# zfountas/deep-active-inference-mc

Hardware: AMD Instinct MI355X
Metric: EFE rollouts/sec (64x64 dSprites, 10 MC-samples, depth 5) (higher is better)
Workload: dtype f32; 1 GPU; calculate_G_repeated: 128 rows (32 roots x 4 actions) x depth 5 x 10 MC samples per GPU (BASELINE configs[1]) + action posterior; rows_per_gpu=128, samples=10, depth=5, parallelism=episodes sharded x1, weights replicated

## Files before the change

deep-active-inference-mc_amd/csrc/decoder.hip:

```cpp
#include <utility>
#include "mfma_pipe.h"

namespace efe {

template <class F, int... I> __device__ __forceinline__ void static_for_(F&& f, std::integer_sequence<int, I...>) { (f(std::integral_constant<int, I>{}), ...); }
template <int N, class F> __device__ __forceinline__ void static_for(F&& f) { static_for_(f, std::make_integer_sequence<int, N>{}); }

__host__ __device__ constexpr int w3_nch(int G) { return G == 4 ? 5 : 4; }
__host__ __device__ constexpr int w3_prod(int G, int c) {
    return G < 4 ? 5 * ((G >> 1) + 2 * (c >> 1)) + (G & 1) + 2 * (c & 1)
         : G == 4 ? (c < 2 ? 5 * (1 + 2 * c) + 4 : c < 4 ? 20 + 1 + 2 * (c - 2) : 24)
                  : (c < 2 ? 5 * (2 * c) + 4 : 20 + 2 * (c - 2));
}
__host__ __device__ constexpr bool w3_direct(int pp) { return f22_o1(pp / 5) < 0 && f22_o1(pp % 5) < 0; }
__host__ __device__ constexpr int w3_view(int pp) { return 3 * f22_view(pp / 5) + f22_view(pp % 5); }
__host__ __device__ constexpr int w3_mat(int pp) { return 4 * f22_wt(pp / 5) + f22_wt(pp % 5); }
__host__ __device__ constexpr bool w3_hits(int pp, int o) {
    const int r = o >> 2, c = o & 3, pr = pp / 5, pc = pp % 5;
    return (r == f22_o0(pr) || r == f22_o1(pr)) && (c == f22_o0(pc) || c == f22_o1(pc));
}
__host__ __device__ constexpr bool w3_seen(int G, int c, int o) {
    for (int g = 0; g < G; ++g)
        for (int k = 0; k < w3_nch(g); ++k) if (w3_hits(w3_prod(g, k), o)) return true;
    if (!w3_direct(w3_prod(G, c)))
        for (int k = 0; k < w3_nch(G); ++k)
            if ((w3_direct(w3_prod(G, k)) || k < c) && w3_hits(w3_prod(G, k), o)) return true;
    return false;
}
__host__ __device__ constexpr bool w3_uses_view(int G, int vi) {
    for (int k = 0; k < w3_nch(G); ++k) if (w3_view(w3_prod(G, k)) == vi) return true;
    return false;
}
__host__ __device__ constexpr bool f22_in(int a, int r) { return a == 0 ? r <= 1 : (a == 1 ? r == 1 : r >= 1); }
__host__ __device__ constexpr bool w3_reads(int G, int r, int c) {
    for (int vi = 0; vi < 9; ++vi) if (w3_uses_view(G, vi) && f22_in(vi / 3, r) && f22_in(vi % 3, c)) return true;
    return false;
}

template <int PD, bool LATE, bool OPAQUE, bool WRAP, class WF, class PX, class Piece>
__device__ __forceinline__ void f22_contract(f32x4 (&acc)[16], f32x4 (&aq)[PD][5], const f32x4 bias4, WF wf, PX px, Piece piece) {
    constexpr int NST = 24;
    auto sub = [](const f32x4 a, const f32x4 b) -> f32x4 { if constexpr (OPAQUE) return sub4(a, b); else return a - b; };
    auto add = [](const f32x4 a, const f32x4 b) -> f32x4 { if constexpr (OPAQUE) return add4(a, b); else return a + b; };
    auto view = [&](const f32x4 (&x)[9], int vi) -> f32x4 {
        const int va = vi / 3, vb = vi % 3;
        auto cv = [&](int i) -> f32x4 { return vb == 0 ? sub(x[3 * i], x[3 * i + 1]) : (vb == 1 ? x[3 * i + 1] : sub(x[3 * i + 2], x[3 * i + 1])); };
        return va == 0 ? sub(cv(0), cv(1)) : (va == 1 ? cv(1) : sub(cv(2), cv(1)));
    };
    const f32x4 zero4 = {};
    f32x4 tq[5], xr[9];
    static_for<9>([&](auto i) { if constexpr (w3_reads(0, i / 3, i % 3)) xr[i] = px(i / 3, i % 3, 0); });
    auto add_tmp = [&](auto gg) {
        constexpr int GG = decltype(gg)::value;
        static_for<w3_nch(GG)>([&](auto c) {
            constexpr int PP = w3_prod(GG, c);
            if constexpr (!w3_direct(PP))
                static_for<16>([&](auto o) {
                    if constexpr (w3_hits(PP, o)) {
                        if constexpr (w3_seen(GG, c, o)) acc[o] = add(acc[o], tq[c]);
                        else acc[o] = add(bias4, tq[c]);
                    }
                });
        });
    };
    static_for<NST>([&](auto stc) {
        constexpr int ST = decltype(stc)::value, G = ST >> 2, KC = ST & 3, GN = (ST + 1) >> 2, KN = (ST + 1) & 3;
        constexpr int SP = (ST + PD) % NST, GP = SP >> 2, KP = SP & 3;
        f32x4 vw[9], ac[5];
        static_for<9>([&](auto vi) { if constexpr (w3_uses_view(G, vi)) vw[vi] = view(xr, vi); });
#pragma unroll
        for (int c = 0; c < 5; ++c) ac[c] = aq[ST % PD][c];
        if constexpr (WRAP || ST + PD < NST)
            static_for<w3_nch(GP)>([&](auto c) { aq[ST % PD][c] = wf(w3_mat(w3_prod(GP, c)), KP, ST + PD >= NST); });
        if constexpr (ST + 1 < NST)
            static_for<9>([&](auto i) { if constexpr (w3_reads(GN, i / 3, i % 3)) xr[i] = px(i / 3, i % 3, KN); });
        if constexpr (LATE && KC == 0 && ST > 0) {
            __builtin_amdgcn_sched_barrier(0);
            add_tmp(std::integral_constant<int, (ST > 0 ? G - 1 : 0)>{});
        }
        prio_matrix();
        __builtin_amdgcn_sched_barrier(0);
#pragma unroll
        for (int e = 0; e < 4; ++e)
            static_for<w3_nch(G)>([&](auto c) {
                constexpr int PP = w3_prod(G, c);
                const float b = vw[w3_view(PP)][e], av = ac[c][e];
                if constexpr (w3_direct(PP)) {
                    constexpr int O = 4 * f22_o0(PP / 5) + f22_o0(PP % 5);
                    constexpr bool FIRST = KC == 0 && !w3_seen(G, c, O);
                    acc[O] = __builtin_amdgcn_mfma_f32_16x16x4f32(av, b, (FIRST && e == 0) ? bias4 : acc[O], 0, 0, 0);
                } else {
                    tq[c] = __builtin_amdgcn_mfma_f32_16x16x4f32(av, b, (KC == 0 && e == 0) ? zero4 : tq[c], 0, 0, 0);
                }
            });
        prio_nonmatrix();
        if constexpr (!LATE && KC == 3) add_tmp(std::integral_constant<int, G>{});
        piece(stc);
    });
    if constexpr (LATE) add_tmp(std::integral_constant<int, 5>{});
}

constexpr int DA_PS = 17;
constexpr int DA_BIAS = 273 * DA_PS;

__host__ __device__ constexpr int wino_i0(int a) { return a == 0 ? 0 : (a == 2 ? 2 : 1); }
__host__ __device__ constexpr int wino_i1(int a) { return a == 0 ? 2 : (a == 1 ? 2 : (a == 2 ? 1 : 3)); }
__host__ __device__ constexpr float wino_s1(int a) { return a == 1 ? 1.0f : -1.0f; }
__host__ __device__ constexpr float wino_at(int r, int a) { return r == 0 ? (a < 3 ? 1.0f : 0.0f) : (a == 0 ? 0.0f : (a == 1 ? 1.0f : -1.0f)); }

__device__ __forceinline__ float4 fma4(float s, const float4& x, const float4& y) {
    return make_float4(__builtin_fmaf(s, x.x, y.x), __builtin_fmaf(s, x.y, y.y), __builtin_fmaf(s, x.z, y.z), __builtin_fmaf(s, x.w, y.w));
}
template <int NR, int R0, int MASK>
__device__ __forceinline__ void wino_otrans(f32x16 (&out)[NR][2], const int a, const int b, const f32x16& m) {
#pragma unroll
    for (int r = 0; r < NR; ++r) {
        if (!((MASK >> r) & 1)) continue;
        const float car = wino_at(R0 + r, a);
#pragma unroll
        for (int c = 0; c < 2; ++c) {
            const float cbc = wino_at(c, b);
            if (cbc == 0.0f) continue;
            const float cf = car * cbc;
#pragma unroll
            for (int e = 0; e < 16; ++e) out[r][c][e] = __builtin_fmaf(cf, m[e], out[r][c][e]);
        }
    }
}
template <int NR, int R0, class Pix>
__device__ __forceinline__ void wino_l1(f32x16 (&out)[NR][2], const float4* __restrict__ U, const float4* sm, const int h,
                                        const int mt_, Pix pix) {
    constexpr int PD = 4;
    const unsigned ln = (threadIdx.x & 63u) * 16u;
    const __amdgpu_buffer_rsrc_t ur = wrsrc(U);
    int mt = mt_; asm volatile("" : "+s"(mt));
    constexpr int a_lo = NR == 2 ? 0 : R0, a_hi = NR == 2 ? 4 : R0 + 3;
    auto ufrag = [&](int a, int b, int kc) { return wfrag(ur, ln, (size_t)(((4 * a + b) * 2 + mt) * 8 + kc) * 64); };
    auto bases = [&](int a, int b, int (&pb)[4]) {
        const int i0 = wino_i0(a), i1 = wino_i1(a), j0 = wino_i0(b), j1 = wino_i1(b);
        pb[0] = pix(i0, j0); pb[1] = pix(i0, j1); pb[2] = pix(i1, j0); pb[3] = pix(i1, j1);
    };
    float4 aq[PD], raw[4];
    int pb[4];
#pragma unroll
    for (int p = 0; p < PD; ++p) aq[p] = ufrag(a_lo, 0, p);
    bases(a_lo, 0, pb);
#pragma unroll
    for (int q = 0; q < 4; ++q) raw[q] = sm[pb[q] + h];
    f32x16 xacc;
    const f32x16 zero = {};
    auto xi_row = [&](int a, auto mask) {
        const float s1 = wino_s1(a);
        const int an = a + 1 < a_hi ? a + 1 : a;
#pragma unroll
        for (int b = 0; b < 4; ++b) {
            const float t1 = wino_s1(b);
#pragma unroll
            for (int kc = 0; kc < 8; ++kc) {
                const float4 av = aq[kc % PD];
                aq[kc % PD] = (b * 8 + kc + PD < 32) ? ufrag(a, (b * 8 + kc + PD) >> 3, (kc + PD) & 7) : ufrag(an, 0, (kc + PD) & 7);
                const float4 c0 = fma4(s1, raw[2], raw[0]), c1 = fma4(s1, raw[3], raw[1]);
                const float4 v = fma4(t1, c1, c0);
                if (kc < 7) {
#pragma unroll
                    for (int q = 0; q < 4; ++q) raw[q] = sm[pb[q] + 2 * (kc + 1) + h];
                } else {
                    if (b < 3) bases(a, b + 1, pb);
                    else bases(an, 0, pb);
#pragma unroll
                    for (int q = 0; q < 4; ++q) raw[q] = sm[pb[q] + h];
                }
                prio_matrix();
                __builtin_amdgcn_sched_barrier(0);
                f32x16& x = xacc;
                x = __builtin_amdgcn_mfma_f32_32x32x2f32(av.x, v.x, kc == 0 ? zero : x, 0, 0, 0);
                x = __builtin_amdgcn_mfma_f32_32x32x2f32(av.y, v.y, x, 0, 0, 0);
                x = __builtin_amdgcn_mfma_f32_32x32x2f32(av.z, v.z, x, 0, 0, 0);
                x = __builtin_amdgcn_mfma_f32_32x32x2f32(av.w, v.w, x, 0, 0, 0);
                prio_nonmatrix();
            }
            wino_otrans<NR, R0, decltype(mask)::value>(out, a, b, xacc);
        }
    };
    if constexpr (NR == 2) {
        xi_row(0, std::integral_constant<int, 1>{});
#pragma unroll 1
        for (int a = 1; a < 3; ++a) xi_row(a, std::integral_constant<int, 3>{});
        xi_row(3, std::integral_constant<int, 2>{});
    } else {
#pragma unroll 1
        for (int a = a_lo; a < a_hi; ++a) xi_row(a, std::integral_constant<int, 1>{});
    }
}
template <class Pix>
__device__ __forceinline__ void wino_l1_rows(f32x16 (&out)[2][2], const float4* __restrict__ U, const float4* sm, const int h,
                                             const int mt_, Pix pix) {
    const unsigned ln = (threadIdx.x & 63u) * 16u;
    const __amdgpu_buffer_rsrc_t ur = wrsrc(U);
    int mt = mt_; asm volatile("" : "+s"(mt));
    auto ufrag = [&](int a, int b, int kc) { return wfrag(ur, ln, (size_t)(((4 * a + b) * 2 + mt) * 8 + kc) * 64); };
    auto bases = [&](int a, int (&pb)[8]) {
#pragma unroll
        for (int jj = 0; jj < 4; ++jj) { pb[jj] = pix(wino_i0(a), jj); pb[4 + jj] = pix(wino_i1(a), jj); }
    };
    float4 aq[4], raw[8];
    int pb[8];
#pragma unroll
    for (int b = 0; b < 4; ++b) aq[b] = ufrag(0, b, 0);
    bases(0, pb);
#pragma unroll
    for (int q = 0; q < 8; ++q) raw[q] = sm[pb[q] + h];
    f32x16 xacc[4];
    const f32x16 zero = {};
    auto xi_row = [&](int a, auto mask) {
        const float s1 = wino_s1(a);
        const int an = a + 1 < 4 ? a + 1 : a;
#pragma unroll
        for (int kc = 0; kc < 8; ++kc) {
            float4 av[4], col[4], v[4];
#pragma unroll
            for (int b = 0; b < 4; ++b) { av[b] = aq[b]; aq[b] = kc < 7 ? ufrag(a, b, kc + 1) : ufrag(an, b, 0); }
#pragma unroll
            for (int jj = 0; jj < 4; ++jj) col[jj] = fma4(s1, raw[4 + jj], raw[jj]);
#pragma unroll
            for (int b = 0; b < 4; ++b) v[b] = fma4(wino_s1(b), col[wino_i1(b)], col[wino_i0(b)]);
            if (kc == 7) bases(an, pb);
#pragma unroll
            for (int q = 0; q < 8; ++q) raw[q] = sm[pb[q] + (kc < 7 ? 2 * (kc + 1) : 0) + h];
            prio_matrix();
            __builtin_amdgcn_sched_barrier(0);
#pragma unroll
            for (int b = 0; b < 4; ++b) {
                f32x16& x = xacc[b];
                x = __builtin_amdgcn_mfma_f32_32x32x2f32(av[b].x, v[b].x, kc == 0 ? zero : x, 0, 0, 0);
                x = __builtin_amdgcn_mfma_f32_32x32x2f32(av[b].y, v[b].y, x, 0, 0, 0);
                x = __builtin_amdgcn_mfma_f32_32x32x2f32(av[b].z, v[b].z, x, 0, 0, 0);
                x = __builtin_amdgcn_mfma_f32_32x32x2f32(av[b].w, v[b].w, x, 0, 0, 0);
                if (b < 3) __builtin_amdgcn_sched_barrier(0);
            }
            prio_nonmatrix();
        }
#pragma unroll
        for (int b = 0; b < 4; ++b) {
            wino_otrans<2, 0, decltype(mask)::value>(out, a, b, xacc[b]);
            __builtin_amdgcn_sched_barrier(0);
        }
    };
    xi_row(0, std::integral_constant<int, 1>{});
#pragma unroll 1
    for (int a = 1; a < 3; ++a) xi_row(a, std::integral_constant<int, 3>{});
    xi_row(3, std::integral_constant<int, 2>{});
}
struct F22Nb { int xb, c2[3], r2; };
__device__ __forceinline__ F22Nb f22_nb(const int xb, const int zq, const int bv, const int bu) {
    F22Nb nb;
    nb.xb = xb;
    nb.c2[0] = bv == 7 ? zq : xb + 2 * DA_PS;
    nb.c2[1] = bv == 7 ? zq : xb + 18 * DA_PS;
    nb.c2[2] = (bv == 7 || bu == 7) ? zq : xb + 34 * DA_PS;
    nb.r2 = bu == 7 ? zq : xb + 32 * DA_PS;
    return nb;
}
__device__ __forceinline__ f32x4 f22_wfrag(const __amdgpu_buffer_rsrc_t wr, const unsigned ln, int ct, int m, int kc) {
    return __builtin_bit_cast(f32x4, wfrag(wr, ln + (unsigned)kc * 1024u, (size_t)(m * 4 + ct) * 256));
}
constexpr int F22_PD = 2;
__device__ __forceinline__ void f22_l2_first(f32x4 (&aq)[F22_PD][5], const __amdgpu_buffer_rsrc_t wr, const int dn, const unsigned ln) {
    static_for<F22_PD>([&](auto p) {
        static_for<w3_nch(p >> 2)>([&](auto c) { aq[p][c] = f22_wfrag(wr, ln, dn, w3_mat(w3_prod(p >> 2, c)), p & 3); });
    });
}
template <bool LATE = false>
__device__ __forceinline__ void f22_l2(f32x4 (&acc)[16], f32x4 (&aq)[F22_PD][5], const __amdgpu_buffer_rsrc_t wr, const int dn,
                                       const unsigned ln, const f32x4 bias4, const f32x4* smv, const F22Nb& nb) {
    auto px = [&](int i, int jj, int kc) -> f32x4 {
        return smv[(jj == 2 ? nb.c2[i] : (i == 2 ? nb.r2 + jj * DA_PS : nb.xb + (16 * i + jj) * DA_PS)) + 4 * kc];
    };
    f22_contract<F22_PD, LATE, false, true>(acc, aq, bias4, [&](int m, int kc, bool next) { return f22_wfrag(wr, ln, next ? dn : 0, m, kc); }, px, [](auto) {});
}
__device__ __forceinline__ void f22_l2_store(f32x4 (&acc)[16], const __amdgpu_buffer_rsrc_t yr, const unsigned yoff, const int ct, const bool on) {
#pragma unroll
    for (int orow = 0; orow < 4; ++orow)
#pragma unroll
        for (int c = 0; c < 2; ++c) {
            u32x4 lo, hi;
#pragma unroll
            for (int e = 0; e < 4; ++e) {
                const unsigned x0 = __builtin_bit_cast(unsigned, relu_nan(acc[4 * orow + c][e]));
                const unsigned x1 = __builtin_bit_cast(unsigned, relu_nan(acc[4 * orow + c + 2][e]));
                const auto sw = __builtin_amdgcn_permlane32_swap(x0, x1, false, false);
                lo[e] = sw[0]; hi[e] = sw[1];
            }
            const unsigned so = (unsigned)(((2 * (orow & 1) + c) * 4096 + 2 * ct * 512 + (orow >> 1) * 32) * 16);
            if (on) {
                __builtin_amdgcn_raw_buffer_store_b128(lo, yr, yoff, so, 0);
                __builtin_amdgcn_raw_buffer_store_b128(hi, yr, yoff, so + 512u * 16u, 0);
            }
        }
}

template <class T>
__device__ __forceinline__ T karg_reload(const int kp_lo, const int kp_hi, const size_t offset) {
    const unsigned long long base = ((unsigned long long)(unsigned)__builtin_amdgcn_readfirstlane(kp_hi) << 32) | (unsigned)__builtin_amdgcn_readfirstlane(kp_lo);
    const __attribute__((address_space(4))) char* p = (const __attribute__((address_space(4))) char*)base + offset;
    T t;
    __builtin_memcpy(&t, reinterpret_cast<const __attribute__((address_space(4))) T*>(p), sizeof(T));
    return t;
}

__device__ __forceinline__ int vpark(int x) { asm volatile("" : "+v"(x)); return x; }
__device__ __forceinline__ int vscalar(int x) { return __builtin_amdgcn_readfirstlane(x); }

__device__ __forceinline__ void dec_a_load_x4(f32x4 (&pf)[16], const float* x4, const int pimg, const int w, const int tl, const int lo, const int hi) {
    const __amdgpu_buffer_rsrc_t xr = wrsrc(x4 + (size_t)pimg * 16384);
#pragma unroll
    for (int it = 0; it < 16; ++it)
        if (it >= lo && it < hi) pf[it] = __builtin_bit_cast(f32x4, wfrag(xr, (unsigned)(w * 16384 + (tl & 63) * 16 + (it & 3) * 1024), (size_t)(it >> 2) * 256));
}

template <bool FUSED, class Tail>
__device__ __forceinline__ void dec_a_loop(const DecAArgs& a_, float4* const sm, Tail&& tail, const int kp_lo = 0, const int kp_hi = 0) {
    const DecAArgs& a = a_;
    constexpr int NTHR = 256;
    constexpr int NPH = 2048 / NTHR;
    constexpr int NPE = 8;
    const int tid = threadIdx.x;
    const int lane = tid & 63;
    const int w_ = __builtin_amdgcn_readfirstlane(tid >> 6);

    if ((int)blockIdx.x >= a.rows) return;
    int* const slot = reinterpret_cast<int*>(sm + DA_BIAS + 32);
    if (tid == 0) slot[0] = 2 * (int)gridDim.x + atomicAdd(a.queue, 1);
    int nimg = (int)blockIdx.x + (int)gridDim.x;
    f32x4 pf[2 * NPH];
    f32x4* smv = reinterpret_cast<f32x4*>(sm);
    {
        const f32x4* X = reinterpret_cast<const f32x4*>(a.x4) + (size_t)blockIdx.x * 4096;
#pragma unroll
        for (int it = 0; it < 2 * NPH; ++it) pf[it] = X[w_ * 1024 + it * 64 + lane];
    }
    if constexpr (!FUSED)
        for (int i = tid; i < 17 * DA_PS; i += NTHR) sm[256 * DA_PS + i] = make_float4(0.f, 0.f, 0.f, 0.f);
    if (tid < 16) sm[DA_BIAS + tid] = reinterpret_cast<const float4*>(a.b1)[tid];
    else if (tid < 32) sm[DA_BIAS + tid] = reinterpret_cast<const float4*>(a.b2)[tid - 16];

    const int rows_v = FUSED ? vpark(a_.rows) : 0, bx_v = FUSED ? vpark((int)blockIdx.x) : 0;
    if constexpr (FUSED) nimg = vpark(nimg);
    for (int img = FUSED ? vpark((int)blockIdx.x) : (int)blockIdx.x; (FUSED ? vscalar(img) : img) < (FUSED ? vscalar(rows_v) : a_.rows);) {
        DecAArgs ai;
        if constexpr (FUSED) ai = karg_reload<DecAArgs>(kp_lo, kp_hi, 0);
        const DecAArgs& a = FUSED ? ai : a_;
        const float4* W1 = reinterpret_cast<const float4*>(a.w1);
        const float4* W2 = reinterpret_cast<const float4*>(a.w2);
        int tl_ = tid; asm volatile("" : "+v"(tl_));
        const int j = tl_ & 31, h = (tl_ >> 5) & 1;
        const int w = FUSED ? __builtin_amdgcn_readfirstlane(tl_ >> 6) : w_;
        const bool live = FUSED ? __builtin_amdgcn_readfirstlane((int)row_live(a.live, vscalar(img))) != 0 : row_live(a.live, img);
        if (live) {
            const int sbase = (64 * w + ((tl_ >> 4) & 3)) * DA_PS + (tl_ & 15);
#pragma unroll
            for (int it = 0; it < 2 * NPH; ++it) smv[sbase + it * 4 * DA_PS] = pf[it];
        }
        if constexpr (FUSED)
            for (int i = tl_; i < 17 * DA_PS; i += NTHR) sm[256 * DA_PS + i] = make_float4(0.f, 0.f, 0.f, 0.f);
        __syncthreads();
        const int nnimg = slot[0];
        int ticket = 0;
        if ((FUSED ? tl_ : tid) == 0) ticket = 2 * (int)gridDim.x + atomicAdd(a.queue, 1);
        const int l1mt = w >> 1, l1n = 32 * (w & 1) + j;
        const int l1y = 2 * (l1n >> 3) - 1, l1x = 2 * (l1n & 7) - 1;
        if (live) {
            f32x16 l1o[2][2];
#pragma unroll
            for (int g4 = 0; g4 < 4; ++g4) {
                const float4 bb = sm[DA_BIAS + l1mt * 8 + 2 * g4 + h];
#pragma unroll
                for (int rc = 0; rc < 4; ++rc) { l1o[rc >> 1][rc & 1][4 * g4] = bb.x; l1o[rc >> 1][rc & 1][4 * g4 + 1] = bb.y; l1o[rc >> 1][rc & 1][4 * g4 + 2] = bb.z; l1o[rc >> 1][rc & 1][4 * g4 + 3] = bb.w; }
            }
            auto l1pix = [&](int i, int jj) {
                const int y = l1y + i, x = l1x + jj;
                return ((unsigned)y < 16u && (unsigned)x < 16u ? y * 16 + x : 256) * DA_PS;
            };
            if constexpr (FUSED) wino_l1_rows(l1o, W1, sm, h, l1mt, l1pix);
            else wino_l1<2, 0>(l1o, W1, sm, h, l1mt, l1pix);
            __syncthreads();
            if ((FUSED ? tl_ : tid) == 0) slot[0] = ticket;
#pragma unroll
            for (int rc = 0; rc < 4; ++rc) {
                const int pix = (l1y + 1 + (rc >> 1)) * 16 + l1x + 1 + (rc & 1);
#pragma unroll
                for (int g4 = 0; g4 < 4; ++g4) {
                    const f32x16& o = l1o[rc >> 1][rc & 1];
                    float4 v;
                    v.x = relu_nan(o[4 * g4 + 0]); v.y = relu_nan(o[4 * g4 + 1]);
                    v.z = relu_nan(o[4 * g4 + 2]); v.w = relu_nan(o[4 * g4 + 3]);
                    sm[pix * DA_PS + l1mt * 8 + 2 * g4 + h] = v;
                }
            }
        } else {
            __syncthreads();
            if ((FUSED ? tl_ : tid) == 0) slot[0] = ticket;
        }
        __syncthreads();
        {
            int t2_ = tid; asm volatile("" : "+v"(t2_));
            const int n = t2_ & 15, g = (t2_ >> 4) & 3;
            const int bu = 2 * w + (n >> 3), bv = n & 7;
            const F22Nb nb = f22_nb((32 * bu + 2 * bv) * DA_PS + g, 256 * DA_PS + g, bv, 0);
            const unsigned ln = (unsigned)(t2_ & 63) * 16u;
            const unsigned yoff = (unsigned)(((32 * bu + 2 * bv + (g >> 1)) * 2 + (g & 1)) * 16);
            const __amdgpu_buffer_rsrc_t yr = wrsrc(a.y2 + (size_t)(FUSED ? vscalar(bx_v) : __builtin_amdgcn_readfirstlane(img)) * (32 * 32 * 64));
            auto load_next = [&](const int lo, const int hi) {
                const int pimg = __builtin_amdgcn_readfirstlane(nimg < a.rows ? nimg : img);
                dec_a_load_x4(pf, a.x4, pimg, w, t2_, lo, hi);
            };
            if (live) {
                f32x4 aq[F22_PD][5], acc2[16];
                f22_l2_first(aq, wrsrc(W2), 0, ln);
                if constexpr (!FUSED) load_next(0, NPE);
#pragma unroll 1
                for (int ct = 0; ct < 4; ++ct) {
                    const f32x4 bias4 = smv[DA_BIAS + 16 + 4 * ct + g];
                    f22_l2<FUSED>(acc2, aq, wrsrc(W2 + ct * 256), ct < 3 ? 1 : 0, ln, bias4, smv, nb);
                    if (ct < 3) f22_l2_store(acc2, yr, yoff, ct, true);
                }
                if constexpr (!FUSED) load_next(NPE, 2 * NPH);
                f22_l2_store(acc2, yr, yoff, 3, true);
                if constexpr (FUSED) tail(img, nimg, pf);
            } else {
                load_next(0, 2 * NPH);
            }
        }
        __syncthreads();
        img = nimg; nimg = FUSED ? vpark(nnimg) : nnimg;
    }
}

__global__ void __launch_bounds__(256, 2) k_dec_a(const DecAArgs a) {
    extern __shared__ __attribute__((aligned(16))) float4 sm[];
    dec_a_loop<false>(a, sm, [](int, int, f32x4 (&)[16]) {});
}

constexpr int DAS_IN = 6 * 16;
constexpr int DAS_L1 = 4 * 16;
constexpr int DAS_BIAS = (DAS_IN + 1 + DAS_L1 + 2) * DA_PS;
constexpr size_t DAS_LDS_BYTES = (DAS_BIAS + 32) * sizeof(float4);
__global__ void __launch_bounds__(256, 2) k_dec_a_s(const DecAArgs a) {
    extern __shared__ __attribute__((aligned(16))) float4 sm[];
    float4* sin = sm;
    float4* sl1 = sm + (DAS_IN + 1) * DA_PS;
    const int tid = threadIdx.x, lane = tid & 63;
    const int w = __builtin_amdgcn_readfirstlane(tid >> 6);
    const int j = lane & 31, h = lane >> 5;
    const int img = blockIdx.x >> 3, p = blockIdx.x & 7;
    if (!row_live(a.live, img)) return;
    const float4* W1 = reinterpret_cast<const float4*>(a.w1);
    const float4* W2 = reinterpret_cast<const float4*>(a.w2);
    {
        const float4* X = reinterpret_cast<const float4*>(a.x4) + (size_t)img * 4096;
        const int c4 = tid & 15, px0 = tid >> 4;
        float4 v[6];
#pragma unroll
        for (int it = 0; it < 6; ++it) {
            const int pix = px0 + 16 * it, lr = pix >> 4, y = 2 * p - 1 + lr;
            v[it] = (y >= 0 && y < 16) ? X[(y * 16 + (pix & 15)) * 16 + c4] : make_float4(0.f, 0.f, 0.f, 0.f);
        }
#pragma unroll
        for (int it = 0; it < 6; ++it) sin[(px0 + 16 * it) * DA_PS + c4] = v[it];
    }
    if (tid < 16) sin[DAS_IN * DA_PS + tid] = make_float4(0.f, 0.f, 0.f, 0.f);
    if (tid < 2 * DA_PS) sl1[DAS_L1 * DA_PS + tid] = make_float4(0.f, 0.f, 0.f, 0.f);
    if (tid < 16) sm[DAS_BIAS + tid] = reinterpret_cast<const float4*>(a.b1)[tid];
    else if (tid < 32) sm[DAS_BIAS + tid] = reinterpret_cast<const float4*>(a.b2)[tid - 16];
    __syncthreads();
    const int mt = w >> 1;
    {
        const int r = w & 1, n = j & 15;
        const int ly = 2 * (n >> 3) - 1, lx = 2 * (n & 7) - 1;
        f32x16 o[1][2];
#pragma unroll
        for (int g4 = 0; g4 < 4; ++g4) {
            const float4 bb = sm[DAS_BIAS + mt * 8 + 2 * g4 + h];
#pragma unroll
            for (int c = 0; c < 2; ++c) { o[0][c][4 * g4] = bb.x; o[0][c][4 * g4 + 1] = bb.y; o[0][c][4 * g4 + 2] = bb.z; o[0][c][4 * g4 + 3] = bb.w; }
        }
        auto pix = [&](int i, int jj) {
            const int sy = ly + 1 + i, x = lx + jj, y = 2 * p - 1 + sy;
            return ((unsigned)y < 16u && (unsigned)x < 16u ? sy * 16 + x : DAS_IN) * DA_PS;
        };
        if (r) wino_l1<1, 1>(o, W1, sin, h, mt, pix);
        else wino_l1<1, 0>(o, W1, sin, h, mt, pix);
        if (j < 16)
#pragma unroll
        for (int c = 0; c < 2; ++c)
#pragma unroll
            for (int g4 = 0; g4 < 4; ++g4) {
                float4 v;
                v.x = relu_nan(o[0][c][4 * g4 + 0]); v.y = relu_nan(o[0][c][4 * g4 + 1]);
                v.z = relu_nan(o[0][c][4 * g4 + 2]); v.w = relu_nan(o[0][c][4 * g4 + 3]);
                sl1[((ly + 1 + r) * 16 + lx + 1 + c) * DA_PS + mt * 8 + 2 * g4 + h] = v;
            }
    }
    __syncthreads();
    {
        const int n = lane & 15, g = lane >> 4, bv = n & 7;
        const F22Nb nb = f22_nb(2 * bv * DA_PS + g, DAS_L1 * DA_PS + g, bv, p);
        const unsigned ln = (unsigned)lane * 16u;
        const unsigned yoff = (unsigned)(((32 * p + 2 * bv + (g >> 1)) * 2 + (g & 1)) * 16);
        const __amdgpu_buffer_rsrc_t yr = wrsrc(a.y2 + (size_t)img * (32 * 32 * 64));
        const __amdgpu_buffer_rsrc_t wr = wrsrc(W2 + w * 256);
        f32x4 aq[F22_PD][5], acc2[16];
        f22_l2_first(aq, wr, 0, ln);
        const f32x4 bias4 = reinterpret_cast<const f32x4*>(sm)[DAS_BIAS + 16 + 4 * w + g];
        f22_l2(acc2, aq, wr, 0, ln, bias4, reinterpret_cast<const f32x4*>(sl1), nb);
        f22_l2_store(acc2, yr, yoff, w, n < 8);
    }
}

constexpr size_t DA_LDS_BYTES = (DA_BIAS + 33) * sizeof(float4);
int init_dec_b_kernels();
int init_decoder_kernels() {
    if (hipFuncSetAttribute((const void*)k_dec_a, hipFuncAttributeMaxDynamicSharedMemorySize, DA_LDS_BYTES) != hipSuccess) return 1;
    if (hipFuncSetAttribute((const void*)k_dec_a_s, hipFuncAttributeMaxDynamicSharedMemorySize, DAS_LDS_BYTES) != hipSuccess) return 1;
    return init_dec_b_kernels();
}

void launch_dec_a(const DecAArgs& a, hipStream_t st) {
    if (a.parts == 8) {
        hipLaunchKernelGGL(k_dec_a_s, dim3(a.rows * 8), dim3(256), DAS_LDS_BYTES, st, a);
        return;
    }
    const size_t lds = DA_LDS_BYTES;
    const int grid = a.rows < 512 ? a.rows : 512;
    hipLaunchKernelGGL(k_dec_a, dim3(grid), dim3(256), lds, st, a);
}


template <int PARTS, bool FUSED>
__device__ __forceinline__ void dec_b_image(const DecBArgs& a, float4* const sm, float4* const sb3, float* const sq, float* const sQ,
                                            const int img, const int qtr, const float* const y2img) {
    constexpr int SR = 4, NW = 4, NTHR = 256;
    constexpr int DB_RP = 33;
    constexpr int DB_PS = 17;
    constexpr int DB_IN_F4 = (SR + 1) * DB_RP * DB_PS;
    constexpr int DB_YROWS = 4 * SR + 2;
    constexpr int NPF = (SR + 1) * 512 / NTHR;
    constexpr int NS = 32 / SR;
    float* sH = reinterpret_cast<float*>(sm + DB_IN_F4);
    int tid = threadIdx.x;
    if constexpr (FUSED) asm volatile("" : "+v"(tid));
    const int lane = tid & 63;
    const int w = __builtin_amdgcn_readfirstlane(tid >> 6);
    const int g = lane >> 4, v = lane & 15;
    const int u = w >> 1, hf = w & 1;
    constexpr int parts = PARTS;
    const int s_lo = parts == 1 ? 0 : (qtr ? 2 * qtr - 1 : 0);
    const int s_hi = parts == 1 ? NS : 2 * qtr + 2;

    const int mg = a.m0 + img;
    const int gi = mg / a.rows_per_group;
    const int r = mg - gi * a.rows_per_group;
    int gt, gp, gs;
    group_decode(a.gm, gi, gt, gp, gs);
    const int mode = (gp == 0 && a.reward0) ? 1 : 0;
    const int slot = (gp == 0 && a.store0) ? gt * a.gm.S + gs : -1;
    float* po = (slot >= 0) ? a.po + ((size_t)slot * a.rows_per_group + r) * 4096 : nullptr;
    int mode_v = mode, mg_v = mg, ri_v = a.reward_intent;
    float* valp = a.val;
    if constexpr (FUSED) { asm volatile("" : "+v"(po)); asm volatile("" : "+v"(valp)); mode_v = vpark(mode_v); mg_v = vpark(mg_v); ri_v = vpark(ri_v); }

    if constexpr (!FUSED) { if (tid < 8) sb3[tid] = reinterpret_cast<const float4*>(a.b3)[tid]; }
    if (tid < (SR + 1) * 16) sm[((tid >> 4) * DB_RP + 32) * DB_PS + (tid & 15)] = make_float4(0.f, 0.f, 0.f, 0.f);
    f32x4 w4a;
    {
        const int kh = v >> 2, kw = v & 3;
#pragma unroll
        for (int rr = 0; rr < 4; ++rr) w4a[rr] = (kh < 3 && kw < 3) ? a.w4[(3 * kh + kw) * 32 + 16 * hf + 4 * g + rr] : 0.f;
    }

    const __amdgpu_buffer_rsrc_t xr_ = __builtin_amdgcn_make_buffer_rsrc(const_cast<float*>(y2img), 0, 32 * 32 * 64 * 4, 0x00020000);
    const unsigned long long y2a = (unsigned long long)y2img;
    const int y2lo_v = FUSED ? vpark((int)(unsigned)y2a) : 0, y2hi_v = FUSED ? vpark((int)(unsigned)(y2a >> 32)) : 0;
    const __amdgpu_buffer_rsrc_t wr = wrsrc(a.w3 + (size_t)hf * 4 * 64 * 4);
    const unsigned ln = (unsigned)lane * 16u;
    auto wf = [&](int m, int kc, bool) -> f32x4 {
        return __builtin_bit_cast(f32x4, FUSED ? wfrag(wr, ln + (unsigned)kc * 1024u, (size_t)(m * 8) * 64) : wfrag(wr, ln, (size_t)(m * 8 + kc) * 64));
    };
    const float D1 = 1.00001f, D0 = 0.00001f;
    float part = 0.f;
    f32x4 pf[NPF];
    f32x4* smv = reinterpret_cast<f32x4*>(sm);
    auto prefetch = [&](int sn, int tl) {
        const __amdgpu_buffer_rsrc_t xr = !FUSED ? xr_ : __builtin_amdgcn_make_buffer_rsrc(
            reinterpret_cast<float*>(((unsigned long long)(unsigned)vscalar(y2hi_v) << 32) | (unsigned)vscalar(y2lo_v)), 0, 32 * 32 * 64 * 4, 0x00020000);
        const unsigned lo = (unsigned)(((tl >> 5) * 512 + (tl & 31)) * 16);
        const unsigned lh = lo | (sn == NS - 1 ? 0x80000000u : 0u);
#pragma unroll
        for (int it = 0; it < NPF; ++it) {
            const int rl = it >> 1;
            const unsigned pc = (unsigned)((((rl & 1) * 16 + (it & 1) * 8) * 512 + (rl >> 1) * 32) * 16);
            pf[it] = __builtin_bit_cast(f32x4, __builtin_amdgcn_raw_buffer_load_b128(xr, rl == SR ? lh : lo, pc + (unsigned)sn * 1024u, 0));
        }
    };
    prefetch(s_lo, tid);

    const int xb = (2 * u * DB_RP + 2 * v) * DB_PS + g;
    auto px = [&](int i, int jj, int kc) -> f32x4 { return smv[xb + (i * DB_RP + jj) * DB_PS + 4 * kc]; };

    constexpr int RWG = 2 * SR / NW;
    float gh[RWG][6], gpr[RWG];
    constexpr unsigned HROW = 2 * 3 * 64 * sizeof(float), HRING = DB_YROWS * HROW;
    auto ring_fwd = [&](unsigned o, unsigned rows) { o += rows * HROW; const unsigned t = o - HRING; return t < o ? t : o; };
    const float* const sHl = sH + lane;
    unsigned gm[RWG][3];
    auto g_load = [&](unsigned go, int q) {
#pragma unroll
        for (int kh = 0; kh < 3; ++kh) {
            const float* hq = reinterpret_cast<const float*>(reinterpret_cast<const char*>(sHl) + (kh == 2 ? go : ring_fwd(go, 2 - kh))) + kh * 64;
            gh[q][2 * kh] = hq[0]; gh[q][2 * kh + 1] = hq[3 * 64];
        }
    };
    auto g_mask = [&](int oh, int q) {
#pragma unroll
        for (int kh = 0; kh < 3; ++kh) gm[q][kh] = (unsigned)(oh + 1 - kh) <= 63u ? ~0u : 0u;
    };
    auto g_sig = [&](int q) {
        float val = a.b4;
#pragma unroll
        for (int kh = 0; kh < 3; ++kh)
            val = add1(val, __builtin_bit_cast(float, __builtin_bit_cast(unsigned, add1(gh[q][2 * kh], gh[q][2 * kh + 1])) & gm[q][kh]));
        gpr[q] = hw_sigmoid(val);
    };
    auto g_term = [&](int oh, int q) {
#pragma clang fp contract(off)
        const float pr = gpr[q];
        const float l1 = hw_log(D1 - pr), l0 = hw_log(D0 + pr);
        const float te = __builtin_fmaf(pr - 1.0f, l1, -(pr * l0));
        const float tw = reward_term(pr, oh, lane, 64, 64, ri_v);
        const float t = mode_v == 0 ? te : tw;
        part += oh >= 0 ? t : 0.0f;
    };
    auto g_store = [&](int oh, int q) {
        if (po && oh >= 0) {
            int owl = lane; asm volatile("" : "+v"(owl));
            (po + oh * 64)[owl] = gpr[q];
        }
    };

    auto fold = [&](int k) { sq[k * NTHR + tid] = part; part = 0.f; };
    char* const sHw = reinterpret_cast<char*>(sH + hf * (3 * 64) + g * 64 + 4 * v);
    unsigned hbo = 0;
    const int tl = tid;
    f32x4* const sp = smv + ((tl & 31) >> 1) * (2 * DB_PS) + 2 * (tl >> 5) + (tl & 1);
    for (int s = s_lo; s < s_hi; ++s) {
        const bool gq = parts == 1 ? true : s == 2 * qtr + 1;
        const int oh0 = 2 * SR * (s - 1) - 1 + w, oh1 = oh0 + NW;
        const unsigned go0 = ring_fwd(hbo, DB_YROWS - 2 * SR - 2 + w), go1 = ring_fwd(go0, NW);
        const unsigned hwo = ring_fwd(hbo, 4 * u);
        g_mask(oh0, 0); g_mask(oh1, 1);
        {
#pragma unroll
            for (int it = 0; it < NPF; ++it) sp[((it >> 1) * DB_RP + (it & 1)) * DB_PS] = pf[it];
        }
        f32x4 aq[1][5];
#pragma unroll
        for (int c = 0; c < w3_nch(0); ++c) aq[0][c] = wf(w3_mat(w3_prod(0, c)), 0, false);
        __syncthreads();

        const f32x4 bias4 = __builtin_bit_cast(f32x4, sb3[4 * hf + g]);
        const f32x4 zero4 = {};
        f32x4 acc[16];
        f22_contract<1, true, true, false>(acc, aq, bias4, wf, px, [&](auto stc) {
            constexpr int ST = decltype(stc)::value;
            if (gq) {
                if constexpr (ST == 0) { g_load(go0, 0); g_load(go1, 1); }
                if constexpr (ST == 2) g_sig(0);
                if constexpr (ST == 5) g_term(oh0, 0);
                if constexpr (ST == 8) g_sig(1);
                if constexpr (ST == 11) g_term(oh1, 1);
            }
        });
        if (!(FUSED && s == NS - 1)) prefetch((s < NS - 1) ? s + 1 : NS - 1, tl);
        auto relu_row = [&](int orow) {
#pragma unroll
            for (int oc = 0; oc < 4; ++oc)
#pragma unroll
                for (int e = 0; e < 4; ++e) acc[4 * orow + oc][e] = relu_nan(acc[4 * orow + oc][e]);
        };
        auto presum_row = [&](const f32x4 (&T)[4], int orow) {
            f32x4 hv;
            hv[0] = add1(add1(T[1][0], T[0][1]), dpp_shr1_zero(T[3][2]));
            hv[1] = add1(add1(T[2][0], T[1][1]), T[0][2]);
            hv[2] = add1(add1(T[3][0], T[2][1]), T[1][2]);
            hv[3] = add1(add1(dpp_shl1_zero(T[0][0]), T[3][1]), T[2][2]);
            if (g < 3) *reinterpret_cast<f32x4*>(sHw + ring_fwd(hwo, orow)) = hv;
        };
        f32x4 T[2][4];
        relu_row(0);
#pragma unroll
        for (int orow = 0; orow < 4; ++orow) {
            __builtin_amdgcn_sched_barrier(0);
#pragma unroll
            for (int e = 0; e < 4; ++e)
#pragma unroll
                for (int oc = 0; oc < 4; ++oc)
                    T[orow & 1][oc] = __builtin_amdgcn_mfma_f32_16x16x4f32(w4a[e], acc[4 * orow + oc][e], e == 0 ? zero4 : T[orow & 1][oc], 0, 0, 0);
            if (orow < 3) relu_row(orow + 1);
            if (orow > 0) presum_row(T[(orow - 1) & 1], orow - 1);
        }
        __builtin_amdgcn_sched_barrier(0);
        presum_row(T[1], 3);
        __syncthreads();
        if (gq) { g_store(oh0, 0); g_store(oh1, 1); }
        if (parts == 1 && (s == 2 || s == 4 || s == 6)) fold(s / 2 - 1);
        if (s == s_hi - 1) {
#pragma unroll
            for (int q = 0; q <= RWG; ++q) {
                if (q == RWG && (w != 0 || s != NS - 1)) break;
                const int oh = 2 * SR * s - 1 + q * NW + w;
                g_mask(oh, 0);
                g_load(ring_fwd(ring_fwd(hbo, DB_YROWS - 2), q * NW + w), 0); g_sig(0); g_term(oh, 0); g_store(oh, 0);
            }
        }
        hbo = ring_fwd(hbo, 2 * SR);
    }
    fold(parts == 1 ? 3 : 0);
    __syncthreads();
    if (w < (parts == 1 ? 4 : 1)) {
        const float* qk = sq + w * NTHR + lane;
        float val = add1(add1(qk[0], qk[64]), add1(qk[128], qk[192]));
#pragma unroll
        for (int o = 32; o > 0; o >>= 1) val += __shfl_xor(val, o);
        if (lane == 0) sQ[w] = val;
    }
    __syncthreads();
    if (tid == 0) {
        if (parts == 1) valp[mg_v] = add1(add1(sQ[0], sQ[1]), add1(sQ[2], sQ[3]));
        else a.valq[(size_t)mg * 4 + qtr] = sQ[0];
    }
}

template <int PARTS>
__global__ void __launch_bounds__(256, 2) k_dec_b4(const DecBArgs a) {
    extern __shared__ __attribute__((aligned(16))) float4 sm[];
    __shared__ float4 sb3[8];
    __shared__ float sq[4 * 256];
    __shared__ float sQ[4];
    const int img = PARTS == 1 ? (int)blockIdx.x : (int)(blockIdx.x >> 2);
    const int qtr = PARTS == 1 ? 0 : (int)(blockIdx.x & 3);
    if (!row_live(a.live, img)) return;
    dec_b_image<PARTS, false>(a, sm, sb3, sq, sQ, img, qtr, a.y2 + (size_t)img * (32 * 32 * 64));
}

constexpr size_t DB_LDS4D = ((5 * 33) * 17) * sizeof(float4) + 18 * 2 * 3 * 64 * sizeof(float);

constexpr int DAB_SB3 = DA_BIAS + 33, DAB_SQ = DAB_SB3 + 8, DAB_SQQ = DAB_SQ + 256;
constexpr size_t DAB_LDS_BYTES = (DAB_SQQ + 1) * sizeof(float4);
static_assert(DB_LDS4D <= DA_BIAS * sizeof(float4), "k_dec_b4's strips and ring must not reach k_dec_a's biases and ticket slot");
static_assert(DAB_LDS_BYTES <= 80 * 1024, "two workgroups of k_dec_ab per CU");
__global__ void __launch_bounds__(256, 2) k_dec_ab(const DecABArgs a) {
    __shared__ __attribute__((aligned(16))) float4 sm[DAB_SQQ + 1];
    float4* const sb3 = sm + DAB_SB3;
    float* const sq = reinterpret_cast<float*>(sm + DAB_SQ);
    float* const sQ = reinterpret_cast<float*>(sm + DAB_SQQ);
    if (threadIdx.x < 8) sb3[threadIdx.x] = reinterpret_cast<const float4*>(a.b.b3)[threadIdx.x];
    const unsigned long long kp = (unsigned long long)__builtin_amdgcn_kernarg_segment_ptr();
    const int kp_lo = vpark((int)(unsigned)kp), kp_hi = vpark((int)(unsigned)(kp >> 32));
    dec_a_loop<true>(a.a, sm, [&](const int img, const int nimg, f32x4 (&pf)[16]) {
        asm volatile("s_waitcnt vmcnt(0)" ::: "memory");
        __syncthreads();
        const DecBArgs b = karg_reload<DecBArgs>(kp_lo, kp_hi, __builtin_offsetof(DecABArgs, b));
        dec_b_image<1, true>(b, sm, sb3, sq, sQ, __builtin_amdgcn_readfirstlane(img), 0, b.y2 + (size_t)vscalar(vpark((int)blockIdx.x)) * (32 * 32 * 64));
        const DecAArgs an = karg_reload<DecAArgs>(kp_lo, kp_hi, 0);
        int tl = threadIdx.x; asm volatile("" : "+v"(tl));
        const int pimg = __builtin_amdgcn_readfirstlane(nimg < an.rows ? nimg : img);
        dec_a_load_x4(pf, an.x4, pimg, __builtin_amdgcn_readfirstlane(tl >> 6), tl, 0, 16);
    }, kp_lo, kp_hi);
}

int init_dec_b_kernels() {
    if (hipFuncSetAttribute((const void*)k_dec_b4<1>, hipFuncAttributeMaxDynamicSharedMemorySize, DB_LDS4D) != hipSuccess) return 1;
    if (hipFuncSetAttribute((const void*)k_dec_b4<4>, hipFuncAttributeMaxDynamicSharedMemorySize, DB_LDS4D) != hipSuccess) return 1;
    return 0;
}

int dec_ab_grid(int rows, int cap) { const int g = rows < 512 ? rows : 512; return cap > 0 && cap < g ? cap : g; }
void launch_dec_ab(const DecABArgs& a, int grid_cap, hipStream_t st) {
    hipLaunchKernelGGL(k_dec_ab, dim3(dec_ab_grid(a.a.rows, grid_cap)), dim3(256), 0, st, a);
}

void launch_dec_b(const DecBArgs& a, hipStream_t st) {
    if (a.parts == 4) hipLaunchKernelGGL(k_dec_b4<4>, dim3(a.rows * 4), dim3(256), DB_LDS4D, st, a);
    else hipLaunchKernelGGL(k_dec_b4<1>, dim3(a.rows), dim3(256), DB_LDS4D, st, a);
}

__host__ __device__ inline int fc4_spg(int mtiles) { return ((mtiles + 7) / 8 + 7) / 8; }
template <int NT>
__global__ void __launch_bounds__(256, 2) k_fc4(const GemmArgs a) {
    constexpr int RT = 32 * NT;
    extern __shared__ __attribute__((aligned(16))) float4 sm[];
    const int tid = threadIdx.x;
    const int lane = tid & 63;
    const int w = __builtin_amdgcn_readfirstlane(tid >> 6);
    const int j = lane & 31, h = lane >> 5;
    const int fgrp = blockIdx.x & 7;
    const int nper = gridDim.x >> 3, k = blockIdx.x >> 3;
    const int SPG = fc4_spg(a.mtiles);
    const int nsteps = ((a.n_pix + RT - 1) / RT) * SPG;
    const int q0 = (int)(((long)nsteps * k) / nper), q1 = (int)(((long)nsteps * (k + 1)) / nper);
    f32x4* smv = reinterpret_cast<f32x4*>(sm);
    const float4* Wl = reinterpret_cast<const float4*>(a.Wp);
    auto xaddr = [&](int t, int (&bs)[NT], int (&sw)[NT], int& wt) {
        wt = t;
#pragma unroll
        for (int nt = 0; nt < NT; ++nt) { bs[nt] = (nt * 32 + j) * 64 + t * 16; sw[nt] = j & 15; }
    };
    int cur_rt = -1;
    uint32_t krow[2] = {0, 0}, kstream[2] = {0, 0}, kstage[2] = {0, 0};
    bool rv[2] = {false, false};
#pragma unroll 1
    for (int q = q0; q < q1; ++q) {
        const int rt = q / SPG, fs = q - rt * SPG;
        const int row0 = rt * RT;
        if (rt != cur_rt) {
            if (cur_rt >= 0) __syncthreads();
            cur_rt = rt;
            const f32x4* X = reinterpret_cast<const f32x4*>(a.X);
#pragma unroll
            for (int it = 0; it < 8 * NT; ++it) {
                const int idx = it * 256 + tid;
                const int r = idx >> 6, c4 = idx & 63;
                const int gr = row0 + r;
                smv[r * 64 + (c4 ^ (r & 15))] = (gr < a.n_pix) ? X[(size_t)gr * 64 + c4] : (f32x4)(0.f);
            }
            __syncthreads();
#pragma unroll
            for (int nt = 0; nt < NT; ++nt) {
                const int m = row0 + nt * 32 + j;
                rv[nt] = m < a.n_pix;
                const int mg = a.m0 + (rv[nt] ? m : 0);
                const int g = mg / a.rows_per_group;
                krow[nt] = global_row(a.gm.ids, a.gm.ids_div, mg - g * a.rows_per_group, a.row_offset);
                const uint2 key = group_key(a.gm, g);
                kstream[nt] = key.x; kstage[nt] = key.y;
            }
        }
        const int mt0 = (fgrp * SPG + fs) * 8 + 2 * w;
        if (mt0 >= a.mtiles) continue;
        f32x16 acc[2][NT];
#pragma unroll
        for (int mt = 0; mt < 2; ++mt)
#pragma unroll
            for (int nt = 0; nt < NT; ++nt)
#pragma unroll
                for (int e = 0; e < 16; ++e) acc[mt][nt][e] = 0.f;
        float4 bq[2][4];
#pragma unroll
        for (int mt = 0; mt < 2; ++mt)
#pragma unroll
            for (int g4 = 0; g4 < 4; ++g4) bq[mt][g4] = *reinterpret_cast<const float4*>(a.bias + (mt0 + mt) * 32 + 8 * g4 + 4 * h);
        tap_loop<2, NT>(acc, 4, Wl, sm, h, xaddr, DenseWIdx{mt0});
#pragma unroll
        for (int nt = 0; nt < NT; ++nt) {
            if (!rv[nt]) continue;
            const uint4 rnd = noise_words(a.k0, a.k1, a.tag, (uint32_t)((mt0 * 32) >> 7), krow[nt], kstream[nt], kstage[nt]);
            float* yp = a.Y + (size_t)(row0 + nt * 32 + j) * a.ldy;
#pragma unroll
            for (int mt = 0; mt < 2; ++mt)
#pragma unroll
                for (int g4 = 0; g4 < 4; ++g4) {
                    const int co = (mt0 + mt) * 32 + 8 * g4 + 4 * h;
                    const float4 bb = bq[mt][g4];
                    const uint32_t word = ((co >> 5) & 3) == 0 ? rnd.x : ((co >> 5) & 3) == 1 ? rnd.y : ((co >> 5) & 3) == 2 ? rnd.z : rnd.w;
                    float v[4] = {acc[mt][nt][4 * g4 + 0] + bb.x, acc[mt][nt][4 * g4 + 1] + bb.y,
                                  acc[mt][nt][4 * g4 + 2] + bb.z, acc[mt][nt][4 * g4 + 3] + bb.w};
#pragma unroll
                    for (int e = 0; e < 4; ++e) v[e] = relu_nan(v[e]) * keep2(((word >> ((co + e) & 31)) & 1u));
                    *reinterpret_cast<float4*>(yp + co) = make_float4(v[0], v[1], v[2], v[3]);
                }
        }
    }
}

void launch_fc4(const GemmArgs& a, hipStream_t st) {
    if (a.n_pix <= 32) {
        const int nsteps = fc4_spg(a.mtiles);
        hipLaunchKernelGGL(k_fc4<1>, dim3(8 * (nsteps < 64 ? nsteps : 64)), dim3(256), 32 * 64 * sizeof(float4), st, a);
        return;
    }
    const int nsteps = ((a.n_pix + 63) / 64) * fc4_spg(a.mtiles);
    const int nper = nsteps < 64 ? nsteps : 64;
    hipLaunchKernelGGL(k_fc4<2>, dim3(8 * nper), dim3(256), 64 * 64 * sizeof(float4), st, a);
}

}
```

Before: 12720 rollouts/s.

## Overlap next-image x4 prefetch with decoder-B tail and cache w4 fragments in LDS

In the fused decoder kernel, the w4 weight fragments are staged once per workgroup in LDS instead of being gathered from global memory for every image. The first w3 fragments are loaded before the initial barrier. Part of the next image's x4 input load is issued during decoder B's final strip instead of after it finishes, and decoder B reuses the caller's prefetch registers rather than keeping its own. The aim is to hide global load latency between the two stages and drop redundant weight reads, at the cost of more LDS per workgroup and more register pressure from holding the extra fragments across the stage boundary.

```diff
diff --git a/deep-active-inference-mc_amd/csrc/decoder.hip b/deep-active-inference-mc_amd/csrc/decoder.hip
--- a/deep-active-inference-mc_amd/csrc/decoder.hip
+++ b/deep-active-inference-mc_amd/csrc/decoder.hip
@@ -536,9 +536,11 @@
 }
 
 
-template <int PARTS, bool FUSED>
+struct DecBNoNext { __device__ __forceinline__ void operator()() const {} };
+template <int PARTS, bool FUSED, class NextX4 = DecBNoNext>
 __device__ __forceinline__ void dec_b_image(const DecBArgs& a, float4* const sm, float4* const sb3, float* const sq, float* const sQ,
-                                            const int img, const int qtr, const float* const y2img) {
+                                            const int img, const int qtr, const float* const y2img,
+                                            const float4* const sw4 = nullptr, f32x4* const pfx = nullptr, NextX4&& next_x4 = NextX4{}) {
     constexpr int SR = 4, NW = 4, NTHR = 256;
     constexpr int DB_RP = 33;
     constexpr int DB_PS = 17;
@@ -570,9 +572,10 @@
     if constexpr (FUSED) { asm volatile("" : "+v"(po)); asm volatile("" : "+v"(valp)); mode_v = vpark(mode_v); mg_v = vpark(mg_v); ri_v = vpark(ri_v); }
 
     if constexpr (!FUSED) { if (tid < 8) sb3[tid] = reinterpret_cast<const float4*>(a.b3)[tid]; }
-    if (tid < (SR + 1) * 16) sm[((tid >> 4) * DB_RP + 32) * DB_PS + (tid & 15)] = make_float4(0.f, 0.f, 0.f, 0.f);
+    if constexpr (!FUSED) { if (tid < (SR + 1) * 16) sm[((tid >> 4) * DB_RP + 32) * DB_PS + (tid & 15)] = make_float4(0.f, 0.f, 0.f, 0.f); }
     f32x4 w4a;
-    {
+    if constexpr (FUSED) w4a = __builtin_bit_cast(f32x4, sw4[hf * 64 + lane]);
+    else {
         const int kh = v >> 2, kw = v & 3;
 #pragma unroll
         for (int rr = 0; rr < 4; ++rr) w4a[rr] = (kh < 3 && kw < 3) ? a.w4[(3 * kh + kw) * 32 + 16 * hf + 4 * g + rr] : 0.f;
@@ -588,7 +591,8 @@
     };
     const float D1 = 1.00001f, D0 = 0.00001f;
     float part = 0.f;
-    f32x4 pf[NPF];
+    f32x4 pfl[FUSED ? 1 : NPF];
+    f32x4* const pf = FUSED ? pfx : pfl;
     f32x4* smv = reinterpret_cast<f32x4*>(sm);
     auto prefetch = [&](int sn, int tl) {
         const __amdgpu_buffer_rsrc_t xr = !FUSED ? xr_ : __builtin_amdgcn_make_buffer_rsrc(
@@ -602,6 +606,14 @@
             pf[it] = __builtin_bit_cast(f32x4, __builtin_amdgcn_raw_buffer_load_b128(xr, rl == SR ? lh : lo, pc + (unsigned)sn * 1024u, 0));
         }
     };
+    f32x4 aqf[1][5];
+    if constexpr (FUSED) {
+        asm volatile("s_waitcnt vmcnt(0)" ::: "memory");
+#pragma unroll
+        for (int c = 0; c < w3_nch(0); ++c) aqf[0][c] = wf(w3_mat(w3_prod(0, c)), 0, false);
+        __syncthreads();
+        if (tid < (SR + 1) * 16) sm[((tid >> 4) * DB_RP + 32) * DB_PS + (tid & 15)] = make_float4(0.f, 0.f, 0.f, 0.f);
+    }
     prefetch(s_lo, tid);
 
     const int xb = (2 * u * DB_RP + 2 * v) * DB_PS + g;
@@ -662,9 +674,12 @@
 #pragma unroll
             for (int it = 0; it < NPF; ++it) sp[((it >> 1) * DB_RP + (it & 1)) * DB_PS] = pf[it];
         }
-        f32x4 aq[1][5];
-#pragma unroll
-        for (int c = 0; c < w3_nch(0); ++c) aq[0][c] = wf(w3_mat(w3_prod(0, c)), 0, false);
+        f32x4 aql[1][5];
+        f32x4 (&aq)[1][5] = FUSED ? aqf : aql;
+        if (!FUSED || s != s_lo) {
+#pragma unroll
+            for (int c = 0; c < w3_nch(0); ++c) aq[0][c] = wf(w3_mat(w3_prod(0, c)), 0, false);
+        }
         __syncthreads();
 
         const f32x4 bias4 = __builtin_bit_cast(f32x4, sb3[4 * hf + g]);
@@ -680,7 +695,8 @@
                 if constexpr (ST == 11) g_term(oh1, 1);
             }
         });
-        if (!(FUSED && s == NS - 1)) prefetch((s < NS - 1) ? s + 1 : NS - 1, tl);
+        if (FUSED && s == NS - 1) next_x4();
+        else prefetch((s < NS - 1) ? s + 1 : NS - 1, tl);
         auto relu_row = [&](int orow) {
 #pragma unroll
             for (int oc = 0; oc < 4; ++oc)
@@ -755,26 +771,36 @@
 constexpr size_t DB_LDS4D = ((5 * 33) * 17) * sizeof(float4) + 18 * 2 * 3 * 64 * sizeof(float);
 
 constexpr int DAB_SB3 = DA_BIAS + 33, DAB_SQ = DAB_SB3 + 8, DAB_SQQ = DAB_SQ + 256;
-constexpr size_t DAB_LDS_BYTES = (DAB_SQQ + 1) * sizeof(float4);
+constexpr int DAB_X4_EARLY = 10;
+constexpr int DAB_W4A = DAB_SQQ + 1;
+constexpr size_t DAB_LDS_BYTES = (DAB_SQQ + 1 + 2 * 64) * sizeof(float4);
 static_assert(DB_LDS4D <= DA_BIAS * sizeof(float4), "k_dec_b4's strips and ring must not reach k_dec_a's biases and ticket slot");
 static_assert(DAB_LDS_BYTES <= 80 * 1024, "two workgroups of k_dec_ab per CU");
 __global__ void __launch_bounds__(256, 2) k_dec_ab(const DecABArgs a) {
-    __shared__ __attribute__((aligned(16))) float4 sm[DAB_SQQ + 1];
+    __shared__ __attribute__((aligned(16))) float4 sm[DAB_SQQ + 1 + 2 * 64];
     float4* const sb3 = sm + DAB_SB3;
     float* const sq = reinterpret_cast<float*>(sm + DAB_SQ);
     float* const sQ = reinterpret_cast<float*>(sm + DAB_SQQ);
     if (threadIdx.x < 8) sb3[threadIdx.x] = reinterpret_cast<const float4*>(a.b.b3)[threadIdx.x];
+    if (threadIdx.x < 2 * 64) {
+        const int hf = threadIdx.x >> 6, g = (threadIdx.x >> 4) & 3, kh = (threadIdx.x >> 2) & 3, kw = threadIdx.x & 3;
+        float4 t = make_float4(0.f, 0.f, 0.f, 0.f);
+        if (kh < 3 && kw < 3) t = *reinterpret_cast<const float4*>(a.b.w4 + (3 * kh + kw) * 32 + 16 * hf + 4 * g);
+        sm[DAB_W4A + threadIdx.x] = t;
+    }
     const unsigned long long kp = (unsigned long long)__builtin_amdgcn_kernarg_segment_ptr();
     const int kp_lo = vpark((int)(unsigned)kp), kp_hi = vpark((int)(unsigned)(kp >> 32));
     dec_a_loop<true>(a.a, sm, [&](const int img, const int nimg, f32x4 (&pf)[16]) {
-        asm volatile("s_waitcnt vmcnt(0)" ::: "memory");
-        __syncthreads();
+        auto next_x4 = [&](const int lo, const int hi) {
+            const DecAArgs an = karg_reload<DecAArgs>(kp_lo, kp_hi, 0);
+            int tl = threadIdx.x; asm volatile("" : "+v"(tl));
+            const int pimg = __builtin_amdgcn_readfirstlane(nimg < an.rows ? nimg : img);
+            dec_a_load_x4(pf, an.x4, pimg, __builtin_amdgcn_readfirstlane(tl >> 6), tl, lo, hi);
+        };
         const DecBArgs b = karg_reload<DecBArgs>(kp_lo, kp_hi, __builtin_offsetof(DecABArgs, b));
-        dec_b_image<1, true>(b, sm, sb3, sq, sQ, __builtin_amdgcn_readfirstlane(img), 0, b.y2 + (size_t)vscalar(vpark((int)blockIdx.x)) * (32 * 32 * 64));
-        const DecAArgs an = karg_reload<DecAArgs>(kp_lo, kp_hi, 0);
-        int tl = threadIdx.x; asm volatile("" : "+v"(tl));
-        const int pimg = __builtin_amdgcn_readfirstlane(nimg < an.rows ? nimg : img);
-        dec_a_load_x4(pf, an.x4, pimg, __builtin_amdgcn_readfirstlane(tl >> 6), tl, 0, 16);
+        dec_b_image<1, true>(b, sm, sb3, sq, sQ, __builtin_amdgcn_readfirstlane(img), 0, b.y2 + (size_t)vscalar(vpark((int)blockIdx.x)) * (32 * 32 * 64),
+                             sm + DAB_W4A, pf, [&] { next_x4(0, DAB_X4_EARLY); });
+        next_x4(DAB_X4_EARLY, 16);
     }, kp_lo, kp_hi);
 }
 
```

After: 12770 rollouts/s (median of 6 runs). Within noise of the previous version (+0.5%).
